# ShardianLabs/EphemeralNet

Measured on AMD Instinct MI355X. Metric: GiB/s ChaCha20-Poly1305 seal+open (device-resident) at 1/2/4/8 MI355X, higher is better.
Workload: dtype u32; 1 GPU; C2: 65536 x 4096 B records, per-record (key, nonce), AEAD seal+open, device-resident; records_per_gpu=65536, record_bytes=4096, lanes_per_record=2, parallelism=records split over 1 GPU(s), no collective

## Files before the change

### ephemeralnet_amd/csrc/enet_device.hpp

```cpp
#pragma once

#include <hip/hip_runtime.h>
#include <stdint.h>

#include "chacha_lockstep_asm.hpp"

namespace enet {

constexpr uint32_t kSigma0 = 0x61707865u, kSigma1 = 0x3320646eu, kSigma2 = 0x79622d32u,
                   kSigma3 = 0x6b206574u;

__device__ __forceinline__ uint32_t rotl(uint32_t v, int s) { return __builtin_rotateleft32(v, s); }

#define ENET_QR(a, b, c, d)                  \
    do {                                     \
        a += b; d ^= a; d = rotl(d, 16);     \
        c += d; b ^= c; b = rotl(b, 12);     \
        a += b; d ^= a; d = rotl(d, 8);      \
        c += d; b ^= c; b = rotl(b, 7);      \
    } while (0)

struct ChachaRecord {
    uint32_t k[8];
    uint32_t n[3];
    uint32_t pre[12];
};

__device__ __forceinline__ void chacha_record_init(ChachaRecord& R, const uint32_t k[8],
                                                   const uint32_t n[3]) {
#pragma unroll
    for (int i = 0; i < 8; ++i) R.k[i] = k[i];
#pragma unroll
    for (int i = 0; i < 3; ++i) R.n[i] = n[i];
    uint32_t a1 = kSigma1, b1 = k[1], c1 = k[5], d1 = n[0];
    uint32_t a2 = kSigma2, b2 = k[2], c2 = k[6], d2 = n[1];
    uint32_t a3 = kSigma3, b3 = k[3], c3 = k[7], d3 = n[2];
    ENET_QR(a1, b1, c1, d1);
    ENET_QR(a2, b2, c2, d2);
    ENET_QR(a3, b3, c3, d3);
    R.pre[0] = a1; R.pre[1] = b1; R.pre[2] = c1; R.pre[3] = d1;
    R.pre[4] = a2; R.pre[5] = b2; R.pre[6] = c2; R.pre[7] = d2;
    R.pre[8] = a3; R.pre[9] = b3; R.pre[10] = c3; R.pre[11] = d3;
}

__device__ __forceinline__ void chacha_block(const ChachaRecord& R, uint32_t counter,
                                             uint32_t x[16]) {
    uint32_t x0 = kSigma0, x4 = R.k[0], x8 = R.k[4], x12 = counter;
    ENET_QR(x0, x4, x8, x12);
    uint32_t x1 = R.pre[0], x5 = R.pre[1], x9 = R.pre[2], x13 = R.pre[3];
    uint32_t x2 = R.pre[4], x6 = R.pre[5], x10 = R.pre[6], x14 = R.pre[7];
    uint32_t x3 = R.pre[8], x7 = R.pre[9], x11 = R.pre[10], x15 = R.pre[11];
    ENET_QR(x0, x5, x10, x15);
    ENET_QR(x1, x6, x11, x12);
    ENET_QR(x2, x7, x8, x13);
    ENET_QR(x3, x4, x9, x14);
#pragma unroll
    for (int i = 1; i < 10; ++i) {
        ENET_QR(x0, x4, x8, x12);
        ENET_QR(x1, x5, x9, x13);
        ENET_QR(x2, x6, x10, x14);
        ENET_QR(x3, x7, x11, x15);
        ENET_QR(x0, x5, x10, x15);
        ENET_QR(x1, x6, x11, x12);
        ENET_QR(x2, x7, x8, x13);
        ENET_QR(x3, x4, x9, x14);
    }
    x[0] = x0 + kSigma0; x[1] = x1 + kSigma1; x[2] = x2 + kSigma2; x[3] = x3 + kSigma3;
    x[4] = x4 + R.k[0]; x[5] = x5 + R.k[1]; x[6] = x6 + R.k[2]; x[7] = x7 + R.k[3];
    x[8] = x8 + R.k[4]; x[9] = x9 + R.k[5]; x[10] = x10 + R.k[6]; x[11] = x11 + R.k[7];
    x[12] = x12 + counter; x[13] = x13 + R.n[0]; x[14] = x14 + R.n[1]; x[15] = x15 + R.n[2];
}

__device__ __forceinline__ void chacha_block2(const ChachaRecord& R, uint32_t ca, uint32_t cb,
                                              uint32_t xa[16], uint32_t xb[16]) {
    uint32_t a0 = kSigma0, a4 = R.k[0], a8 = R.k[4], a12 = ca;
    uint32_t b0 = kSigma0, b4 = R.k[0], b8 = R.k[4], b12 = cb;
    ENET_QR(a0, a4, a8, a12);
    ENET_QR(b0, b4, b8, b12);
    uint32_t a1 = R.pre[0], a5 = R.pre[1], a9 = R.pre[2], a13 = R.pre[3];
    uint32_t a2 = R.pre[4], a6 = R.pre[5], a10 = R.pre[6], a14 = R.pre[7];
    uint32_t a3 = R.pre[8], a7 = R.pre[9], a11 = R.pre[10], a15 = R.pre[11];
    uint32_t b1 = a1, b5 = a5, b9 = a9, b13 = a13;
    uint32_t b2 = a2, b6 = a6, b10 = a10, b14 = a14;
    uint32_t b3 = a3, b7 = a7, b11 = a11, b15 = a15;
    ENET_QR(a0, a5, a10, a15); ENET_QR(b0, b5, b10, b15);
    ENET_QR(a1, a6, a11, a12); ENET_QR(b1, b6, b11, b12);
    ENET_QR(a2, a7, a8, a13);  ENET_QR(b2, b7, b8, b13);
    ENET_QR(a3, a4, a9, a14);  ENET_QR(b3, b4, b9, b14);
#pragma unroll
    for (int i = 1; i < 10; ++i) {
        ENET_QR(a0, a4, a8, a12);  ENET_QR(b0, b4, b8, b12);
        ENET_QR(a1, a5, a9, a13);  ENET_QR(b1, b5, b9, b13);
        ENET_QR(a2, a6, a10, a14); ENET_QR(b2, b6, b10, b14);
        ENET_QR(a3, a7, a11, a15); ENET_QR(b3, b7, b11, b15);
        ENET_QR(a0, a5, a10, a15); ENET_QR(b0, b5, b10, b15);
        ENET_QR(a1, a6, a11, a12); ENET_QR(b1, b6, b11, b12);
        ENET_QR(a2, a7, a8, a13);  ENET_QR(b2, b7, b8, b13);
        ENET_QR(a3, a4, a9, a14);  ENET_QR(b3, b4, b9, b14);
    }
    xa[0] = a0 + kSigma0; xa[1] = a1 + kSigma1; xa[2] = a2 + kSigma2; xa[3] = a3 + kSigma3;
    xa[4] = a4 + R.k[0]; xa[5] = a5 + R.k[1]; xa[6] = a6 + R.k[2]; xa[7] = a7 + R.k[3];
    xa[8] = a8 + R.k[4]; xa[9] = a9 + R.k[5]; xa[10] = a10 + R.k[6]; xa[11] = a11 + R.k[7];
    xa[12] = a12 + ca; xa[13] = a13 + R.n[0]; xa[14] = a14 + R.n[1]; xa[15] = a15 + R.n[2];
    xb[0] = b0 + kSigma0; xb[1] = b1 + kSigma1; xb[2] = b2 + kSigma2; xb[3] = b3 + kSigma3;
    xb[4] = b4 + R.k[0]; xb[5] = b5 + R.k[1]; xb[6] = b6 + R.k[2]; xb[7] = b7 + R.k[3];
    xb[8] = b8 + R.k[4]; xb[9] = b9 + R.k[5]; xb[10] = b10 + R.k[6]; xb[11] = b11 + R.k[7];
    xb[12] = b12 + cb; xb[13] = b13 + R.n[0]; xb[14] = b14 + R.n[1]; xb[15] = b15 + R.n[2];
}

#define ENET_ASM_ADD(x, y) asm volatile("v_add_u32_e32 %0, %0, %1" : "+v"(x) : "v"(y))
#define ENET_ASM_XOR(x, y) asm volatile("v_xor_b32_e32 %0, %0, %1" : "+v"(x) : "v"(y))
#define ENET_ASM_ROT(x, r) asm volatile("v_alignbit_b32 %0, %0, %0, %1" : "+v"(x) : "I"(32 - (r)))

template <bool DIAG>
__device__ __forceinline__ void chacha_half_lockstep(uint32_t x[32]) {
    constexpr int C[4][4] = {{0, 4, 8, 12}, {1, 5, 9, 13}, {2, 6, 10, 14}, {3, 7, 11, 15}};
    constexpr int D[4][4] = {{0, 5, 10, 15}, {1, 6, 11, 12}, {2, 7, 8, 13}, {3, 4, 9, 14}};
    constexpr int R[4] = {16, 12, 8, 7};
#pragma unroll
    for (int k = 0; k < 4; ++k) {
#pragma unroll
        for (int c = 0; c < 8; ++c) {
            const int* q = DIAG ? D[c & 3] : C[c & 3];
            const int o = 16 * (c >> 2);
            if (k % 2 == 0) ENET_ASM_ADD(x[o + q[0]], x[o + q[1]]);
            else ENET_ASM_ADD(x[o + q[2]], x[o + q[3]]);
        }
#pragma unroll
        for (int c = 0; c < 8; ++c) {
            const int* q = DIAG ? D[c & 3] : C[c & 3];
            const int o = 16 * (c >> 2);
            if (k % 2 == 0) ENET_ASM_XOR(x[o + q[3]], x[o + q[0]]);
            else ENET_ASM_XOR(x[o + q[1]], x[o + q[2]]);
        }
#pragma unroll
        for (int c = 0; c < 8; ++c) {
            const int* q = DIAG ? D[c & 3] : C[c & 3];
            const int o = 16 * (c >> 2);
            if (k % 2 == 0) ENET_ASM_ROT(x[o + q[3]], R[k]);
            else ENET_ASM_ROT(x[o + q[1]], R[k]);
        }
#ifndef ENET_LOCK_EVERY
#define ENET_LOCK_EVERY 1
#endif
        if ((k + 1) % ENET_LOCK_EVERY == 0) __builtin_amdgcn_s_barrier();
    }
}

struct NoStepHook {
    __device__ __forceinline__ void operator()(int) const {}
};
template <bool DIAG, class SH = NoStepHook, int BAR = 1>
__device__ __forceinline__ void chacha_half_lockstep2(uint32_t x[32], SH&& sh = SH{}, int base = 0) {
    auto after = [&](int k) {
        asm volatile("" ::: "memory");
        sh(base + k);
        asm volatile("" ::: "memory");
    };
    constexpr bool b0 = BAR == 1, b1 = BAR == 1 || BAR == 2, b2 = BAR == 1, b3 = BAR != 0;
#define ENET_LS_STEP(NAME, B)                               \
    do {                                                    \
        if constexpr (B) asm volatile(NAME ENET_LS_X32(x)); \
        else asm volatile(NAME##_NB ENET_LS_X32(x));        \
    } while (0)
    if constexpr (DIAG) {
        ENET_LS_STEP(ENET_LS_D0, b0);
        after(0);
        ENET_LS_STEP(ENET_LS_D1, b1);
        after(1);
        ENET_LS_STEP(ENET_LS_D2, b2);
        after(2);
        ENET_LS_STEP(ENET_LS_D3, b3);
        after(3);
    } else {
        ENET_LS_STEP(ENET_LS_C0, b0);
        after(0);
        ENET_LS_STEP(ENET_LS_C1, b1);
        after(1);
        ENET_LS_STEP(ENET_LS_C2, b2);
        after(2);
        ENET_LS_STEP(ENET_LS_C3, b3);
        after(3);
    }
#undef ENET_LS_STEP
}

__device__ __forceinline__ void chacha_block2_lockstep(const ChachaRecord& R, uint32_t ca, uint32_t cb,
                                                       uint32_t xa[16], uint32_t xb[16]) {
    uint32_t a0 = kSigma0, a4 = R.k[0], a8 = R.k[4], a12 = ca;
    uint32_t b0 = kSigma0, b4 = R.k[0], b8 = R.k[4], b12 = cb;
    ENET_QR(a0, a4, a8, a12);
    ENET_QR(b0, b4, b8, b12);
    uint32_t x[32];
    x[0] = a0; x[4] = a4; x[8] = a8; x[12] = a12;
    x[16] = b0; x[20] = b4; x[24] = b8; x[28] = b12;
#pragma unroll
    for (int c = 1; c < 4; ++c) {
#pragma unroll
        for (int r = 0; r < 4; ++r) {
            x[c + 4 * r] = R.pre[4 * (c - 1) + r];
            x[16 + c + 4 * r] = R.pre[4 * (c - 1) + r];
        }
    }
    chacha_half_lockstep2<true>(x);
#pragma unroll
    for (int i = 1; i < 10; ++i) {
        chacha_half_lockstep2<false>(x);
        chacha_half_lockstep2<true>(x);
    }
    const uint32_t ff[16] = {kSigma0, kSigma1, kSigma2, kSigma3, R.k[0], R.k[1], R.k[2], R.k[3],
                             R.k[4], R.k[5], R.k[6], R.k[7], 0u, R.n[0], R.n[1], R.n[2]};
#pragma unroll
    for (int i = 0; i < 16; ++i) {
        xa[i] = x[i] + (i == 12 ? ca : ff[i]);
        xb[i] = x[16 + i] + (i == 12 ? cb : ff[i]);
    }
}

constexpr uint32_t M26 = 0x3ffffffu;

struct Pmul {
    uint32_t r[5];
    uint32_t s[5];
};

__device__ __forceinline__ Pmul pmul_make(const uint32_t r[5]) {
    Pmul m;
#pragma unroll
    for (int i = 0; i < 5; ++i) { m.r[i] = r[i]; m.s[i] = r[i] * 5u; }
    return m;
}

__device__ __forceinline__ void pmul(uint32_t h[5], const Pmul& m) {
    const uint64_t h0 = h[0], h1 = h[1], h2 = h[2], h3 = h[3], h4 = h[4];
    uint64_t d0 = h0 * m.r[0] + h1 * m.s[4] + h2 * m.s[3] + h3 * m.s[2] + h4 * m.s[1];
    uint64_t d1 = h0 * m.r[1] + h1 * m.r[0] + h2 * m.s[4] + h3 * m.s[3] + h4 * m.s[2];
    uint64_t d2 = h0 * m.r[2] + h1 * m.r[1] + h2 * m.r[0] + h3 * m.s[4] + h4 * m.s[3];
    uint64_t d3 = h0 * m.r[3] + h1 * m.r[2] + h2 * m.r[1] + h3 * m.r[0] + h4 * m.s[4];
    uint64_t d4 = h0 * m.r[4] + h1 * m.r[3] + h2 * m.r[2] + h3 * m.r[1] + h4 * m.r[0];
    uint32_t c;
    c = (uint32_t)(d0 >> 26); h[0] = (uint32_t)d0 & M26; d1 += c;
    c = (uint32_t)(d1 >> 26); h[1] = (uint32_t)d1 & M26; d2 += c;
    c = (uint32_t)(d2 >> 26); h[2] = (uint32_t)d2 & M26; d3 += c;
    c = (uint32_t)(d3 >> 26); h[3] = (uint32_t)d3 & M26; d4 += c;
    c = (uint32_t)(d4 >> 26); h[4] = (uint32_t)d4 & M26;
    h[0] += c * 5u;
    c = h[0] >> 26; h[0] &= M26; h[1] += c;
}

__device__ __forceinline__ void padd_block(uint32_t h[5], uint32_t w0, uint32_t w1, uint32_t w2,
                                           uint32_t w3, uint32_t hibit) {
    h[0] += w0 & M26;
    h[1] += __builtin_amdgcn_alignbit(w1, w0, 26) & M26;
    h[2] += __builtin_amdgcn_alignbit(w2, w1, 20) & M26;
    h[3] += __builtin_amdgcn_alignbit(w3, w2, 14) & M26;
    h[4] += (w3 >> 8) | (hibit << 24);
}

__device__ __forceinline__ void plimbs(uint32_t out[5], uint32_t w0, uint32_t w1, uint32_t w2,
                                       uint32_t w3) {
    out[0] = w0 & M26;
    out[1] = __builtin_amdgcn_alignbit(w1, w0, 26) & M26;
    out[2] = __builtin_amdgcn_alignbit(w2, w1, 20) & M26;
    out[3] = __builtin_amdgcn_alignbit(w3, w2, 14) & M26;
    out[4] = w3 >> 8;
}

__device__ __forceinline__ void pfinish(const uint32_t hin[5], const uint32_t s[4],
                                        uint32_t tag[4]) {
    uint32_t h0 = hin[0], h1 = hin[1], h2 = hin[2], h3 = hin[3], h4 = hin[4], c;
#pragma unroll
    for (int pass = 0; pass < 2; ++pass) {
        c = h0 >> 26; h0 &= M26; h1 += c;
        c = h1 >> 26; h1 &= M26; h2 += c;
        c = h2 >> 26; h2 &= M26; h3 += c;
        c = h3 >> 26; h3 &= M26; h4 += c;
        c = h4 >> 26; h4 &= M26; h0 += c * 5u;
    }
    c = h0 >> 26; h0 &= M26; h1 += c;
    uint32_t g0 = h0 + 5u; c = g0 >> 26; g0 &= M26;
    uint32_t g1 = h1 + c; c = g1 >> 26; g1 &= M26;
    uint32_t g2 = h2 + c; c = g2 >> 26; g2 &= M26;
    uint32_t g3 = h3 + c; c = g3 >> 26; g3 &= M26;
    uint32_t g4 = h4 + c - (1u << 26);
    const uint32_t use_g = (g4 >> 31) - 1u;
    h0 = (h0 & ~use_g) | (g0 & use_g);
    h1 = (h1 & ~use_g) | (g1 & use_g);
    h2 = (h2 & ~use_g) | (g2 & use_g);
    h3 = (h3 & ~use_g) | (g3 & use_g);
    h4 = (h4 & ~use_g) | (g4 & use_g);
    uint64_t f;
    f = (uint64_t)(h0 | (h1 << 26)) + s[0]; tag[0] = (uint32_t)f;
    f = (uint64_t)((h1 >> 6) | (h2 << 20)) + s[1] + (f >> 32); tag[1] = (uint32_t)f;
    f = (uint64_t)((h2 >> 12) | (h3 << 14)) + s[2] + (f >> 32); tag[2] = (uint32_t)f;
    f = (uint64_t)((h3 >> 18) | (h4 << 8)) + s[3] + (f >> 32); tag[3] = (uint32_t)f;
}

__device__ __forceinline__ void pclamp(uint32_t r[5], uint32_t w0, uint32_t w1, uint32_t w2,
                                       uint32_t w3) {
    plimbs(r, w0 & 0x0fffffffu, w1 & 0x0ffffffcu, w2 & 0x0ffffffcu, w3 & 0x0ffffffcu);
}

struct PolyR32 {
    uint32_t r0, r1, r2, r3, s1, s2, s3;
};

__device__ __forceinline__ PolyR32 polyr32_make(uint32_t w0, uint32_t w1, uint32_t w2, uint32_t w3) {
    PolyR32 R;
    R.r0 = w0 & 0x0fffffffu;
    R.r1 = w1 & 0x0ffffffcu;
    R.r2 = w2 & 0x0ffffffcu;
    R.r3 = w3 & 0x0ffffffcu;
    R.s1 = R.r1 + (R.r1 >> 2);
    R.s2 = R.r2 + (R.r2 >> 2);
    R.s3 = R.r3 + (R.r3 >> 2);
    return R;
}

__device__ __forceinline__ void poly32_block(uint32_t h[5], const PolyR32& R, uint32_t m0,
                                             uint32_t m1, uint32_t m2, uint32_t m3,
                                             uint32_t hibit) {
    unsigned cy;
    const uint32_t a0 = __builtin_addc(h[0], m0, 0u, &cy);
    const uint32_t a1 = __builtin_addc(h[1], m1, cy, &cy);
    const uint32_t a2 = __builtin_addc(h[2], m2, cy, &cy);
    const uint32_t a3 = __builtin_addc(h[3], m3, cy, &cy);
    const uint32_t a4 = h[4] + hibit + cy;
    const uint64_t d0 = (uint64_t)a0 * R.r0 + (uint64_t)a1 * R.s3 + (uint64_t)a2 * R.s2 +
                        (uint64_t)a3 * R.s1;
    const uint64_t e1 = (uint64_t)a0 * R.r1 + (uint64_t)a1 * R.r0 + (uint64_t)a2 * R.s3 +
                        (uint64_t)a3 * R.s2 + (uint64_t)a4 * R.s1;
    const uint64_t e2 = (uint64_t)a0 * R.r2 + (uint64_t)a1 * R.r1 + (uint64_t)a2 * R.r0 +
                        (uint64_t)a3 * R.s3 + (uint64_t)a4 * R.s2;
    const uint64_t e3 = (uint64_t)a0 * R.r3 + (uint64_t)a1 * R.r2 + (uint64_t)a2 * R.r1 +
                        (uint64_t)a3 * R.r0 + (uint64_t)a4 * R.s3;
    const uint32_t x0 = (uint32_t)d0;
    const uint32_t x1 = __builtin_addc((uint32_t)e1, (uint32_t)(d0 >> 32), 0u, &cy);
    const uint32_t c1 = (uint32_t)(e1 >> 32) + cy;
    const uint32_t x2 = __builtin_addc((uint32_t)e2, c1, 0u, &cy);
    const uint32_t c2 = (uint32_t)(e2 >> 32) + cy;
    const uint32_t x3 = __builtin_addc((uint32_t)e3, c2, 0u, &cy);
    const uint32_t c3 = (uint32_t)(e3 >> 32) + cy;
    const uint32_t t4 = a4 * R.r0 + c3;
    const uint32_t f = (t4 >> 2) * 5u;
    h[0] = __builtin_addc(x0, f, 0u, &cy);
    h[1] = __builtin_addc(x1, 0u, cy, &cy);
    h[2] = __builtin_addc(x2, 0u, cy, &cy);
    h[3] = __builtin_addc(x3, 0u, cy, &cy);
    h[4] = (t4 & 3u) + cy;
}

__device__ __forceinline__ void h32_to_limbs(const uint32_t h[5], uint32_t l[5]) {
    l[0] = h[0] & M26;
    l[1] = __builtin_amdgcn_alignbit(h[1], h[0], 26) & M26;
    l[2] = __builtin_amdgcn_alignbit(h[2], h[1], 20) & M26;
    l[3] = __builtin_amdgcn_alignbit(h[3], h[2], 14) & M26;
    l[4] = (h[3] >> 8) | (h[4] << 24);
}

__device__ __forceinline__ void ppow(const uint32_t r[5], uint32_t e, uint32_t x[5]) {
#pragma unroll
    for (int i = 0; i < 5; ++i) x[i] = r[i];
    const Pmul mr = pmul_make(r);
    const int top = 31 - __builtin_clz(e);
    for (int b = top - 1; b >= 0; --b) {
        pmul(x, pmul_make(x));
        if ((e >> b) & 1u) pmul(x, mr);
    }
}

__device__ __forceinline__ uint32_t bswap32(uint32_t v) { return __builtin_bswap32(v); }
__device__ __forceinline__ uint32_t rotr(uint32_t v, int s) { return __builtin_rotateright32(v, s); }

__constant__ static const uint32_t kSha256K[64] = {
    0x428a2f98u, 0x71374491u, 0xb5c0fbcfu, 0xe9b5dba5u, 0x3956c25bu, 0x59f111f1u, 0x923f82a4u,
    0xab1c5ed5u, 0xd807aa98u, 0x12835b01u, 0x243185beu, 0x550c7dc3u, 0x72be5d74u, 0x80deb1feu,
    0x9bdc06a7u, 0xc19bf174u, 0xe49b69c1u, 0xefbe4786u, 0x0fc19dc6u, 0x240ca1ccu, 0x2de92c6fu,
    0x4a7484aau, 0x5cb0a9dcu, 0x76f988dau, 0x983e5152u, 0xa831c66du, 0xb00327c8u, 0xbf597fc7u,
    0xc6e00bf3u, 0xd5a79147u, 0x06ca6351u, 0x14292967u, 0x27b70a85u, 0x2e1b2138u, 0x4d2c6dfcu,
    0x53380d13u, 0x650a7354u, 0x766a0abbu, 0x81c2c92eu, 0x92722c85u, 0xa2bfe8a1u, 0xa81a664bu,
    0xc24b8b70u, 0xc76c51a3u, 0xd192e819u, 0xd6990624u, 0xf40e3585u, 0x106aa070u, 0x19a4c116u,
    0x1e376c08u, 0x2748774cu, 0x34b0bcb5u, 0x391c0cb3u, 0x4ed8aa4au, 0x5b9cca4fu, 0x682e6ff3u,
    0x748f82eeu, 0x78a5636fu, 0x84c87814u, 0x8cc70208u, 0x90befffau, 0xa4506cebu, 0xbef9a3f7u,
    0xc67178f2u};

constexpr uint32_t kShaIV[8] = {0x6a09e667u, 0xbb67ae85u, 0x3c6ef372u, 0xa54ff53au,
                                0x510e527fu, 0x9b05688cu, 0x1f83d9abu, 0x5be0cd19u};

__device__ __forceinline__ uint32_t xor3(uint32_t a, uint32_t b, uint32_t c) {
    return __builtin_amdgcn_bitop3_b32(a, b, c, 0x96);
}

__device__ __forceinline__ void sha256_compress(uint32_t st[8], uint32_t w[16]) {
    uint32_t a = st[0], b = st[1], c = st[2], d = st[3], e = st[4], f = st[5], g = st[6],
             h = st[7];
#pragma unroll
    for (int i = 0; i < 64; ++i) {
        uint32_t wi;
        if (i < 16) {
            wi = w[i];
        } else {
            const uint32_t w15 = w[(i - 15) & 15], w2 = w[(i - 2) & 15];
            const uint32_t s0 = xor3(rotr(w15, 7), rotr(w15, 18), w15 >> 3);
            const uint32_t s1 = xor3(rotr(w2, 17), rotr(w2, 19), w2 >> 10);
            wi = w[i & 15] + s0 + w[(i - 7) & 15] + s1;
            w[i & 15] = wi;
        }
        const uint32_t S1 = xor3(rotr(e, 6), rotr(e, 11), rotr(e, 25));
        const uint32_t ch = __builtin_amdgcn_bitop3_b32(e, f, g, 0xCA);
        const uint32_t t1 = h + S1 + ch + kSha256K[i] + wi;
        const uint32_t S0 = xor3(rotr(a, 2), rotr(a, 13), rotr(a, 22));
        const uint32_t mj = __builtin_amdgcn_bitop3_b32(a, b, c, 0xE8);
        h = g; g = f; f = e; e = d + t1; d = c; c = b; b = a; a = t1 + S0 + mj;
    }
    st[0] += a; st[1] += b; st[2] += c; st[3] += d;
    st[4] += e; st[5] += f; st[6] += g; st[7] += h;
}

template <int N, int M>
__device__ __forceinline__ void extract_bytes(const uint32_t* in, uint32_t off, uint32_t* out) {
    constexpr int W = N + 1;
    uint32_t a[W];
#pragma unroll
    for (int i = 0; i < N; ++i) a[i] = in[i];
    a[N] = 0u;
    const uint32_t k = off >> 2;
#pragma unroll
    for (int b = 32; b >= 1; b >>= 1) {
        if (b > N) continue;
        const bool t = (k & (uint32_t)b) != 0u;
#pragma unroll
        for (int i = 0; i < W; ++i) a[i] = t ? (i + b < W ? a[i + b] : 0u) : a[i];
    }
    const uint32_t sh = off & 3u;
#pragma unroll
    for (int j = 0; j < M; ++j)
        out[j] = __builtin_amdgcn_alignbyte(j + 1 < W ? a[j + 1] : 0u, a[j], sh);
}

__device__ __forceinline__ void load_block(const uint8_t* __restrict__ p, uint32_t n,
                                           uint32_t w[16], bool window_ok = false) {
    if (n >= 64) {
        const uint4* q = reinterpret_cast<const uint4*>(p);
#pragma unroll
        for (int i = 0; i < 4; ++i) {
            const uint4 v = q[i];
            w[4 * i] = v.x; w[4 * i + 1] = v.y; w[4 * i + 2] = v.z; w[4 * i + 3] = v.w;
        }
    } else if (window_ok) {
        const uint32_t nq = n >> 4;
#pragma unroll
        for (int i = 0; i < 16; ++i) w[i] = 0u;
#pragma unroll
        for (int c = 0; c < 3; ++c) {
            if ((uint32_t)c < nq) {
                const uint4 v = reinterpret_cast<const uint4*>(p)[c];
                w[4 * c] = v.x; w[4 * c + 1] = v.y; w[4 * c + 2] = v.z; w[4 * c + 3] = v.w;
            }
        }
        const uint4 v = *reinterpret_cast<const uint4*>(p + n - 16);
        const uint32_t win[4] = {v.x, v.y, v.z, v.w};
        uint32_t ch[4];
        extract_bytes<4, 4>(win, 16u - (n & 15u), ch);
#pragma unroll
        for (int c = 0; c < 4; ++c) {
#pragma unroll
            for (int i = 0; i < 4; ++i) w[4 * c + i] = ((uint32_t)c == nq) ? ch[i] : w[4 * c + i];
        }
    } else {
#pragma unroll
        for (int i = 0; i < 16; ++i) {
            uint32_t v = 0;
#pragma unroll
            for (int b = 0; b < 4; ++b)
                if ((uint32_t)(4 * i + b) < n) v |= (uint32_t)p[4 * i + b] << (8 * b);
            w[i] = v;
        }
    }
}

__device__ __forceinline__ void store_block(uint8_t* __restrict__ p, uint32_t n,
                                            const uint32_t w[16]) {
    if (n >= 64) {
        uint4* q = reinterpret_cast<uint4*>(p);
#pragma unroll
        for (int i = 0; i < 4; ++i)
            q[i] = make_uint4(w[4 * i], w[4 * i + 1], w[4 * i + 2], w[4 * i + 3]);
    } else if (n >= 16) {
        const uint32_t nq = n >> 4;
#pragma unroll
        for (int c = 0; c < 3; ++c)
            if ((uint32_t)c < nq)
                reinterpret_cast<uint4*>(p)[c] =
                    make_uint4(w[4 * c], w[4 * c + 1], w[4 * c + 2], w[4 * c + 3]);
        uint32_t win[4];
        extract_bytes<16, 4>(w, n - 16u, win);
        *reinterpret_cast<uint4*>(p + n - 16) = make_uint4(win[0], win[1], win[2], win[3]);
    } else {
        const uint32_t nw = n >> 2;
#pragma unroll
        for (int i = 0; i < 3; ++i)
            if ((uint32_t)i < nw) *reinterpret_cast<uint32_t*>(p + 4 * i) = w[i];
        const uint32_t lw = nw == 0 ? w[0] : nw == 1 ? w[1] : nw == 2 ? w[2] : w[3];
#pragma unroll
        for (int b = 0; b < 3; ++b)
            if ((uint32_t)b < (n & 3u)) p[4 * nw + b] = (uint8_t)(lw >> (8 * b));
    }
}

__device__ __forceinline__ uint64_t uniform_u64(uint64_t v) {
    return (uint64_t)(uint32_t)__builtin_amdgcn_readfirstlane((uint32_t)v) |
           ((uint64_t)(uint32_t)__builtin_amdgcn_readfirstlane((uint32_t)(v >> 32)) << 32);
}

__device__ __forceinline__ uint32_t ld32(const uint8_t* p) {
    return (uint32_t)p[0] | ((uint32_t)p[1] << 8) | ((uint32_t)p[2] << 16) | ((uint32_t)p[3] << 24);
}

}
```

### ephemeralnet_amd/csrc/stream.hip

```cpp
#include "record_route.hpp"
#include "stream_common.hpp"

namespace enet {

struct StreamSched {
    int dA, dE, sA, sE;
};
__device__ constexpr StreamSched stream_sched(int v) {
    return v == 1 ? StreamSched{1, 2, 2, 2} : v == 2 ? StreamSched{1, 4, 3, 4}
         : v == 3 ? StreamSched{1, 1, 18, 3} : v == 4 ? StreamSched{1, 2, 2, 2}
         : v == 5 ? StreamSched{1, 1, 1, 1} : StreamSched{1, 3, 2, 3};
}
__device__ constexpr int stream_barf(int v) { return v == 4 ? 2 : v == 5 ? 4 : 1; }
__device__ constexpr int stream_stores_after(StreamSched sc) {
    int n = 0;
    for (int s = 0; s < 16; ++s) n += (sc.sA + sc.sE * s >= sc.dA + 15 * sc.dE) ? 1 : 0;
    return n;
}

template <int LOGP, int MODE, int SCHED = 0>
__global__ __launch_bounds__(kStreamWG) void stream_kernel(RecParams p) {
    constexpr StreamSched SC = stream_sched(SCHED);
    constexpr int BARF = stream_barf(SCHED);
    constexpr int kPos = kStreamSteps / BARF;
    constexpr uint32_t P = 1u << LOGP;
    constexpr bool kPoly = (MODE != MODE_XOR);
    __shared__ __attribute__((aligned(16))) uint8_t s_in[kStreamLanes * kRun];
    __shared__ __attribute__((aligned(16))) uint8_t s_out[kStreamLanes * kRun];

    const uint32_t L = (uint32_t)p.uniform_len;
    const bool compute = threadIdx.x < kStreamLanes;
    const uint32_t gid = blockIdx.x * kStreamLanes + (compute ? threadIdx.x : 0u);
    const uint32_t rec = gid >> LOGP;
    const uint32_t j = gid & (P - 1);
#ifdef ENET_TOOLS_BUILD
    const int dbg = p.dbg;
#else
    constexpr int dbg = 0;
#endif
    const bool stamp = (dbg & 16384) && threadIdx.x == 0 && p.tag_out;
    uint64_t* stamps = reinterpret_cast<uint64_t*>(p.tag_out + 16ull * rec);
    if (__builtin_expect(stamp, 0)) {
        stamps[0] = __builtin_amdgcn_s_memrealtime();
        stamps[1] = __builtin_amdgcn_s_memtime();
    }
    const uint64_t i0 = p.in_off[0], o0 = p.out_off[0];
    {
        const bool mine = !compute || (p.in_off[rec] == i0 + (uint64_t)rec * L &&
                                       p.in_off[rec + 1] == i0 + (uint64_t)(rec + 1) * L &&
                                       p.out_off[rec] == o0 + (uint64_t)rec * L &&
                                       p.out_off[rec + 1] == o0 + (uint64_t)(rec + 1) * L);
        if (!__syncthreads_and(mine ? 1 : 0)) {
            if (compute) records_body<LOGP, MODE, FR_NONE, 7>(p);
            return;
        }
    }

    const uint32_t lane = threadIdx.x & 63u;
    const uint32_t wave = __builtin_amdgcn_readfirstlane(threadIdx.x >> 6);
    const uint32_t B = L >> (6 + LOGP);
    const uint32_t S = B >> 1;
    const bool mem = !(dbg & 1);

    if (!compute) {
        const uint32_t m = wave - 8u;
        const uint32_t kk = lane & 7u;
        if (!(dbg & 4096)) __builtin_amdgcn_s_setprio(3);
        uint32_t offA[2], offAB[2];
#pragma unroll
        for (int c = 0; c < 2; ++c) {
            const uint32_t wg0 = blockIdx.x * kStreamLanes + (2u * m + c) * 64u;
            uint32_t o2[2];
#pragma unroll
            for (int i = 0; i < 2; ++i) {
                const uint32_t o = 8u * i + (lane >> 3);
                const uint32_t go = wg0 + o;
                o2[i] = (go >> LOGP) * L + (((go & (P - 1)) * B) << 6) + 16u * (kk ^ slab_sw(o));
            }
            offA[c] = o2[0];
            offAB[c] = o2[1] - o2[0];
        }
        const uint32_t offD = (16u >> LOGP) * L;
        uint32_t offs[16];
#pragma unroll
        for (int s = 0; s < 16; ++s)
            offs[s] = offA[s >> 3] + (uint32_t)(s & 1) * offAB[s >> 3] + (uint32_t)((s & 7) >> 1) * offD;
        auto uni = [](const void* q) {
            const uint64_t v = reinterpret_cast<uintptr_t>(q);
            return (uint64_t)(uint32_t)__builtin_amdgcn_readfirstlane((uint32_t)v) |
                   ((uint64_t)(uint32_t)__builtin_amdgcn_readfirstlane((uint32_t)(v >> 32)) << 32);
        };
        const uint8_t* ibase = reinterpret_cast<const uint8_t*>(uni(p.in + i0));
        uint8_t* obase = reinterpret_cast<uint8_t*>(uni(p.out + o0));
        const uint32_t in_part = (uint32_t)reinterpret_cast<uintptr_t>(s_in) + 2u * m * (64u * kRun);
        const uint8_t* out_part = s_out + 2u * m * (64u * kRun) + 16u * lane;
        auto dma = [&](const uint8_t* base, int s) {
            const uint32_t m0 = in_part + 1024u * (uint32_t)s;
            uint32_t keep;
            if constexpr (SCHED == 14)
                asm volatile("s_mov_b32 %0, m0\n s_mov_b32 m0, %2\n s_nop 0\n global_load_lds_dwordx4 %1, %3\n s_mov_b32 m0, %0"
                             : "=&s"(keep) : "v"(offs[s]), "s"(m0), "s"(base) : "memory");
            else
                asm volatile("s_mov_b32 %0, m0\n s_mov_b32 m0, %2\n s_nop 0\n global_load_lds_dwordx4 %1, %3 nt\n s_mov_b32 m0, %0"
                             : "=&s"(keep) : "v"(offs[s]), "s"(m0), "s"(base) : "memory");
        };
        auto ldsread = [&](int s) {
            return *reinterpret_cast<const uint4*>(out_part + 1024u * (uint32_t)s);
        };
        auto store = [&](uint8_t* base, int s, uint4 v) {
            enet_u32x4 d = {v.x, v.y, v.z, v.w};
            asm volatile("global_store_dwordx4 %0, %1, %2 nt\n s_nop 1"
                         :: "v"(offs[s]), "v"(d), "s"(base) : "memory");
        };
        uint64_t wait_cyc = 0;
        if (mem) {
#pragma unroll
            for (int s = 0; s < 16; ++s) dma(ibase, s);
            asm volatile("s_waitcnt vmcnt(0)" ::: "memory");
        }
        for (uint32_t st = 0; st < S; ++st) {
            stream_barrier();
            const bool more = mem && st + 1 < S && !(dbg & 128), prev = mem && st > 0 && !(dbg & 64);
            const uint8_t* inext = ibase + (size_t)kRun * (st + 1);
            uint8_t* oprev = obase + (size_t)kRun * (st - 1);
            uint4 v = make_uint4(0, 0, 0, 0);
            if (__builtin_expect(prev, 1)) v = ldsread(0);
#pragma unroll
            for (int k = 0; k < kPos; ++k) {
                if (k >= SC.dA && (k - SC.dA) % SC.dE == 0 && (k - SC.dA) / SC.dE < 16) {
                    if (__builtin_expect(more, 1)) dma(inext, (k - SC.dA) / SC.dE);
                }
                if (k >= SC.sA && (k - SC.sA) % SC.sE == 0 && (k - SC.sA) / SC.sE < 16) {
                    const int sl = (k - SC.sA) / SC.sE;
                    if (__builtin_expect(prev, 1)) {
                        store(oprev, sl, v);
                        if (sl < 15) v = ldsread(sl + 1);
                    }
                }
                stream_barrier();
            }
            constexpr int kStoresAfter = stream_stores_after(SC);
            uint64_t tw0 = 0;
            if (__builtin_expect(dbg & 2048, 0)) tw0 = __builtin_amdgcn_s_memtime();
            if (__builtin_expect(prev, 1)) asm volatile("s_waitcnt vmcnt(%0)" :: "n"(kStoresAfter) : "memory");
            else asm volatile("s_waitcnt vmcnt(0)" ::: "memory");
            if (__builtin_expect(dbg & 2048, 0)) wait_cyc += __builtin_amdgcn_s_memtime() - tw0;
        }
        if (__builtin_expect(dbg & 2048, 0) && lane == 0 && p.tag_out)
            reinterpret_cast<uint64_t*>(p.tag_out)[blockIdx.x * 4u + m] = wait_cyc;
        stream_barrier();
        if (S > 0 && mem) {
            uint8_t* olast = obase + (size_t)kRun * (S - 1);
#pragma unroll
            for (int s = 0; s < 16; ++s) store(olast, s, ldsread(s));
        }
        asm volatile("s_waitcnt vmcnt(0)" ::: "memory");
        stream_barrier();
        return;
    }

    const uint32_t msw = slab_sw(lane);
    if (__builtin_expect(stamp, 0)) stamps[2] = __builtin_amdgcn_s_memtime();

    uint32_t kw[8], nw[3];
    {
        const uint32_t* kp = reinterpret_cast<const uint32_t*>(p.keys + (size_t)p.key_stride * rec);
#pragma unroll
        for (int i = 0; i < 8; ++i) kw[i] = kp[i];
        const uint32_t* np = reinterpret_cast<const uint32_t*>(p.nonces + 12ull * rec);
#pragma unroll
        for (int i = 0; i < 3; ++i) nw[i] = np[i];
    }
    ChachaRecord R;
    chacha_record_init(R, kw, nw);
    uint32_t ctr = 1u;
    if (MODE == MODE_XOR)
        ctr = p.counters ? p.counters[(size_t)rec * (p.counter_stride ? p.counter_stride : 1u)] : 0u;
    ctr += j * B;

    uint64_t clk0 = 0, rt0 = 0;
    if (dbg & 256) {
        clk0 = __builtin_amdgcn_s_memtime();
        rt0 = __builtin_amdgcn_s_memrealtime();
    }

    uint32_t h[5] = {0, 0, 0, 0, 0};
    PolyR32 PR{};
    uint32_t pad[4] = {0, 0, 0, 0};
    uint32_t na = 0, aad_len = 0;
    if (kPoly) {
        uint32_t otk[16];
        chacha_block(R, 0u, otk);
        PR = polyr32_make(otk[0], otk[1], otk[2], otk[3]);
        pad[0] = otk[4]; pad[1] = otk[5]; pad[2] = otk[6]; pad[3] = otk[7];
        uint64_t aoff = 0;
        if (p.aad) {
            aoff = p.aad_off[rec];
            aad_len = (uint32_t)(p.aad_off[rec + 1] - aoff);
        }
        na = (aad_len + 15) >> 4;
        if (j == 0) {
            for (uint32_t s = 0; s < na; ++s) {
                const uint8_t* ap = p.aad + aoff + 16ull * s;
                const uint32_t cnt = min(16u, aad_len - 16u * s);
                uint32_t w[4];
#pragma unroll
                for (int i = 0; i < 4; ++i) {
                    uint32_t v = 0;
#pragma unroll
                    for (int b = 0; b < 4; ++b)
                        if ((uint32_t)(4 * i + b) < cnt) v |= (uint32_t)ap[4 * i + b] << (8 * b);
                    w[i] = v;
                }
                poly32_block(h, PR, w[0], w[1], w[2], w[3], 1u);
            }
        }
    }

    const uint32_t ff[16] = {kSigma0, kSigma1, kSigma2, kSigma3, R.k[0], R.k[1], R.k[2], R.k[3],
                             R.k[4], R.k[5], R.k[6], R.k[7], 0u, R.n[0], R.n[1], R.n[2]};
    for (uint32_t st = 0; st < S; ++st) {
        asm volatile("s_waitcnt lgkmcnt(0)" ::: "memory");
        stream_barrier();
        if (__builtin_expect(stamp, 0)) stamps[3 + st] = __builtin_amdgcn_s_memtime();
        uint8_t* myrun = s_in + threadIdx.x * kRun;
        uint32_t w[32];
        if (__builtin_expect(dbg & 32, 0)) {
#pragma unroll
            for (int k = 0; k < 32; ++k) w[k] = k * lane + st;
        } else {
#pragma unroll
            for (int k = 0; k < 8; ++k) {
                const uint4 v = *reinterpret_cast<const uint4*>(myrun + 16u * (k ^ msw));
                w[4 * k] = v.x; w[4 * k + 1] = v.y; w[4 * k + 2] = v.z; w[4 * k + 3] = v.w;
            }
        }
        const uint32_t c0 = ctr + 2u * st;
        uint32_t x[32];
        {
            uint32_t a0 = kSigma0, a4 = R.k[0], a8 = R.k[4], a12 = c0;
            uint32_t b0 = kSigma0, b4 = R.k[0], b8 = R.k[4], b12 = c0 + 1u;
            ENET_QR(a0, a4, a8, a12);
            ENET_QR(b0, b4, b8, b12);
            x[0] = a0; x[4] = a4; x[8] = a8; x[12] = a12;
            x[16] = b0; x[20] = b4; x[24] = b8; x[28] = b12;
#pragma unroll
            for (int c = 1; c < 4; ++c) {
#pragma unroll
                for (int r = 0; r < 4; ++r) {
                    x[c + 4 * r] = R.pre[4 * (c - 1) + r];
                    x[16 + c + 4 * r] = R.pre[4 * (c - 1) + r];
                }
            }
        }
        asm volatile("s_waitcnt lgkmcnt(0)" ::: "memory");
        if (__builtin_expect(dbg & 2, 0)) {
#pragma unroll
            for (int k = 0; k < kPos; ++k) stream_barrier();
        } else {
            chacha_half_lockstep2<true, NoStepHook, BARF>(x);
#pragma unroll
            for (int dr = 1; dr < 10; ++dr) {
                chacha_half_lockstep2<false, NoStepHook, BARF>(x);
                chacha_half_lockstep2<true, NoStepHook, BARF>(x);
            }
        }
        if (MODE == MODE_OPEN && !(dbg & 4)) {
            poly_block64(h, PR, w);
            poly_block64(h, PR, w + 16);
        }
#pragma unroll
        for (int i = 0; i < 16; ++i) {
            w[i] ^= x[i] + (i == 12 ? c0 : ff[i]);
            w[16 + i] ^= x[16 + i] + (i == 12 ? c0 + 1u : ff[i]);
        }
        if (MODE == MODE_SEAL && !(dbg & 4)) {
            poly_block64(h, PR, w);
            poly_block64(h, PR, w + 16);
        }
        uint8_t* myout = s_out + threadIdx.x * kRun;
        if (__builtin_expect(dbg & 32, 0)) {
            uint32_t acc = 0;
#pragma unroll
            for (int k = 0; k < 32; ++k) acc ^= w[k];
            if (acc == 0x9e3779b9u) myout[0] = 1;
        } else {
#pragma unroll
            for (int k = 0; k < 8; ++k)
                *reinterpret_cast<uint4*>(myout + 16u * (k ^ msw)) =
                    make_uint4(w[4 * k], w[4 * k + 1], w[4 * k + 2], w[4 * k + 3]);
        }
    }
    asm volatile("s_waitcnt lgkmcnt(0)" ::: "memory");
    stream_barrier();
    if (__builtin_expect(stamp, 0)) stamps[3 + S] = __builtin_amdgcn_s_memtime();

    if (dbg & (256 | 2048 | 16384)) {
        const uint64_t clk1 = __builtin_amdgcn_s_memtime(), rt1 = __builtin_amdgcn_s_memrealtime();
        if (threadIdx.x == 0 && p.tag_out && !(dbg & (2048 | 16384))) {
            uint64_t* d = reinterpret_cast<uint64_t*>(p.tag_out + 16ull * rec);
            d[0] = clk0; d[1] = rt0; d[2] = clk1; d[3] = rt1;
        }
        stream_barrier();
        if (__builtin_expect(stamp, 0)) {
            stamps[4 + S] = __builtin_amdgcn_s_memtime();
            stamps[5 + S] = __builtin_amdgcn_s_memrealtime();
        }
        return;
    }
    uint32_t diff = 0;
    if (kPoly) {
        const uint32_t nct = L >> 4;
        const uint32_t N = na + nct + 1;
        uint32_t e = 0;
        if (j == P - 1) poly32_block(h, PR, aad_len, 0u, L, 0u, 1u);
        else e = N - 1 - (na + 4 * (j + 1) * B - 1);
        uint32_t l[5];
        h32_to_limbs(h, l);
        if (P > 1) {
            if (e > 0) {
                uint32_t r26[5], xx[5];
                plimbs(r26, PR.r0, PR.r1, PR.r2, PR.r3);
                ppow(r26, e, xx);
                pmul(l, pmul_make(xx));
            }
#pragma unroll
            for (uint32_t o = P >> 1; o >= 1; o >>= 1) {
#pragma unroll
                for (int i = 0; i < 5; ++i) l[i] += __shfl_xor(l[i], (int)o);
            }
        }
        uint32_t tag[4];
        pfinish(l, pad, tag);
        if (MODE == MODE_SEAL) {
            if (j == 0) {
                uint32_t* tp = reinterpret_cast<uint32_t*>(p.tag_out + 16ull * rec);
                tp[0] = tag[0]; tp[1] = tag[1]; tp[2] = tag[2]; tp[3] = tag[3];
            }
        } else {
            const uint32_t* tp = reinterpret_cast<const uint32_t*>(p.tag_in + 16ull * rec);
            diff = (tag[0] ^ tp[0]) | (tag[1] ^ tp[1]) | (tag[2] ^ tp[2]) | (tag[3] ^ tp[3]);
            if (j == 0) p.ok[rec] = diff == 0 ? 1 : 0;
        }
    }
    stream_barrier();
    if (MODE == MODE_OPEN && diff != 0) {
        uint8_t* seg = p.out + o0 + (uint64_t)rec * L + ((uint64_t)j * B << 6);
        for (uint32_t c = 0; c < 4 * B; ++c)
            *reinterpret_cast<uint4*>(seg + 16ull * c) = make_uint4(0, 0, 0, 0);
    }
}

template <int MODE>
static hipError_t launch_stream_mode(const RecParams& p, uint32_t lanes, uint32_t blocks, hipStream_t s) {
    switch (lanes) {
        case 1: hipLaunchKernelGGL((stream_kernel<0, MODE>), dim3(blocks), dim3(kStreamWG), 0, s, p); break;
        case 2:
#ifdef ENET_TOOLS_BUILD
            switch (p.var) {
                case 1: hipLaunchKernelGGL((stream_kernel<1, MODE, 1>), dim3(blocks), dim3(kStreamWG), 0, s, p); break;
                case 2: hipLaunchKernelGGL((stream_kernel<1, MODE, 2>), dim3(blocks), dim3(kStreamWG), 0, s, p); break;
                case 3: hipLaunchKernelGGL((stream_kernel<1, MODE, 3>), dim3(blocks), dim3(kStreamWG), 0, s, p); break;
                case 4: hipLaunchKernelGGL((stream_kernel<1, MODE, 4>), dim3(blocks), dim3(kStreamWG), 0, s, p); break;
                case 5: hipLaunchKernelGGL((stream_kernel<1, MODE, 5>), dim3(blocks), dim3(kStreamWG), 0, s, p); break;
                case 14: hipLaunchKernelGGL((stream_kernel<1, MODE, 14>), dim3(blocks), dim3(kStreamWG), 0, s, p); break;
                default: hipLaunchKernelGGL((stream_kernel<1, MODE>), dim3(blocks), dim3(kStreamWG), 0, s, p); break;
            }
#else
            hipLaunchKernelGGL((stream_kernel<1, MODE>), dim3(blocks), dim3(kStreamWG), 0, s, p);
#endif
            break;
        case 4: hipLaunchKernelGGL((stream_kernel<2, MODE>), dim3(blocks), dim3(kStreamWG), 0, s, p); break;
        case 8: hipLaunchKernelGGL((stream_kernel<3, MODE>), dim3(blocks), dim3(kStreamWG), 0, s, p); break;
        case 16: hipLaunchKernelGGL((stream_kernel<4, MODE>), dim3(blocks), dim3(kStreamWG), 0, s, p); break;
        default: return hipErrorInvalidValue;
    }
    return hipGetLastError();
}

static_assert(kRouteWideWG == kStreamLanes, "record_route.hpp and the streaming kernel disagree on the workgroup");

hipError_t launch_stream(int mode, const RecParams& p, uint32_t lanes, uint32_t blocks, hipStream_t s) {
    switch (mode) {
        case MODE_XOR: return launch_stream_mode<MODE_XOR>(p, lanes, blocks, s);
        case MODE_SEAL: return launch_stream_mode<MODE_SEAL>(p, lanes, blocks, s);
        case MODE_OPEN: return launch_stream_mode<MODE_OPEN>(p, lanes, blocks, s);
        default: return hipErrorInvalidValue;
    }
}

}
```

### ephemeralnet_amd/csrc/stream_common.hpp

```cpp
#pragma once
#include "records_body.hpp"

namespace enet {

constexpr uint32_t kStreamLanes = 512;
constexpr uint32_t kStreamWG = 768;
constexpr int kStreamSteps = 76;

__device__ __forceinline__ void stream_barrier() { asm volatile("s_barrier" ::: "memory"); }

}
```

Before: 912.7 GiB/s.

## Interleave Poly1305 pieces into ChaCha lockstep steps and add wave-priority variants

Adds a PolySpreadHook that breaks each Poly1305 block update into nine pieces and runs them between the ChaCha lockstep quarter-round steps in open mode. The aim is to hide the MAC arithmetic inside the ChaCha schedule instead of running poly_block64 afterwards. It also adds configurable s_setprio variants for the compute and memory waves, plus a debug timing probe. The default build (issue variant 30) keeps the sequential poly path but pins the w registers first; the spread and priority variants are selectable only in tools builds. The cost is extra register pressure and compiler barriers from the pinning.

```diff
diff --git a/ephemeralnet_amd/csrc/enet_device.hpp b/ephemeralnet_amd/csrc/enet_device.hpp
--- a/ephemeralnet_amd/csrc/enet_device.hpp
+++ b/ephemeralnet_amd/csrc/enet_device.hpp
@@ -2,6 +2,9 @@
 
 #include <hip/hip_runtime.h>
 #include <stdint.h>
+
+#include <type_traits>
+#include <utility>
 
 #include "chacha_lockstep_asm.hpp"
 
@@ -150,11 +153,11 @@
 struct NoStepHook {
     __device__ __forceinline__ void operator()(int) const {}
 };
-template <bool DIAG, class SH = NoStepHook, int BAR = 1>
-__device__ __forceinline__ void chacha_half_lockstep2(uint32_t x[32], SH&& sh = SH{}, int base = 0) {
-    auto after = [&](int k) {
+template <bool DIAG, class SH = NoStepHook, int BAR = 1, int BASE = 0>
+__device__ __forceinline__ void chacha_half_lockstep2(uint32_t x[32], SH&& sh = SH{}) {
+    auto after = [&](auto k) {
         asm volatile("" ::: "memory");
-        sh(base + k);
+        sh(std::integral_constant<int, BASE + decltype(k)::value>{});
         asm volatile("" ::: "memory");
     };
     constexpr bool b0 = BAR == 1, b1 = BAR == 1 || BAR == 2, b2 = BAR == 1, b3 = BAR != 0;
@@ -165,22 +168,22 @@
     } while (0)
     if constexpr (DIAG) {
         ENET_LS_STEP(ENET_LS_D0, b0);
-        after(0);
+        after(std::integral_constant<int, 0>{});
         ENET_LS_STEP(ENET_LS_D1, b1);
-        after(1);
+        after(std::integral_constant<int, 1>{});
         ENET_LS_STEP(ENET_LS_D2, b2);
-        after(2);
+        after(std::integral_constant<int, 2>{});
         ENET_LS_STEP(ENET_LS_D3, b3);
-        after(3);
+        after(std::integral_constant<int, 3>{});
     } else {
         ENET_LS_STEP(ENET_LS_C0, b0);
-        after(0);
+        after(std::integral_constant<int, 0>{});
         ENET_LS_STEP(ENET_LS_C1, b1);
-        after(1);
+        after(std::integral_constant<int, 1>{});
         ENET_LS_STEP(ENET_LS_C2, b2);
-        after(2);
+        after(std::integral_constant<int, 2>{});
         ENET_LS_STEP(ENET_LS_C3, b3);
-        after(3);
+        after(std::integral_constant<int, 3>{});
     }
 #undef ENET_LS_STEP
 }
diff --git a/ephemeralnet_amd/csrc/stream.hip b/ephemeralnet_amd/csrc/stream.hip
--- a/ephemeralnet_amd/csrc/stream.hip
+++ b/ephemeralnet_amd/csrc/stream.hip
@@ -12,10 +12,32 @@
          : v == 5 ? StreamSched{1, 1, 1, 1} : StreamSched{1, 3, 2, 3};
 }
 __device__ constexpr int stream_barf(int v) { return v == 4 ? 2 : v == 5 ? 4 : 1; }
+#ifndef ENET_STREAM_ISSUE
+#define ENET_STREAM_ISSUE 30
+#endif
+struct StreamIssue {
+    int prio_old, prio_young, prio_mem, poly;
+};
+__device__ constexpr StreamIssue stream_issue(int v) {
+    int k = -1, poly = 0;
+    if (v >= 20 && v < 28) k = v - 20;
+    else if (v >= 30 && v <= 32) poly = v - 29;
+    if (k < 0) return StreamIssue{0, 0, 3, poly};
+    const int c = k & 3;
+    return StreamIssue{c == 0 ? 0 : c == 3 ? 2 : 1, c == 1 ? 0 : c == 3 ? 2 : 1, (k & 4) ? 2 : 3, poly};
+}
 __device__ constexpr int stream_stores_after(StreamSched sc) {
     int n = 0;
     for (int s = 0; s < 16; ++s) n += (sc.sA + sc.sE * s >= sc.dA + 15 * sc.dE) ? 1 : 0;
     return n;
+}
+
+__device__ __forceinline__ void stream_where(const RecParams& p, int logp, uint32_t wave, uint32_t lane,
+                                             uint64_t t_entry) {
+    if (lane != 0 || !p.tag_out) return;
+    const uint32_t hw = __builtin_amdgcn_s_getreg(4 | (31 << 11));
+    uint32_t* d = reinterpret_cast<uint32_t*>(p.tag_out + 16ull * ((blockIdx.x * kStreamLanes) >> logp) + 16u * wave);
+    d[0] = (uint32_t)t_entry; d[1] = (uint32_t)(t_entry >> 32); d[2] = hw; d[3] = wave;
 }
 
 template <int LOGP, int MODE, int SCHED = 0>
@@ -25,6 +47,7 @@
     constexpr int kPos = kStreamSteps / BARF;
     constexpr uint32_t P = 1u << LOGP;
     constexpr bool kPoly = (MODE != MODE_XOR);
+    constexpr StreamIssue ISS = stream_issue(SCHED < 20 ? ENET_STREAM_ISSUE : SCHED);
     __shared__ __attribute__((aligned(16))) uint8_t s_in[kStreamLanes * kRun];
     __shared__ __attribute__((aligned(16))) uint8_t s_out[kStreamLanes * kRun];
 
@@ -39,6 +62,8 @@
     constexpr int dbg = 0;
 #endif
     const bool stamp = (dbg & 16384) && threadIdx.x == 0 && p.tag_out;
+    uint64_t t_entry = 0;
+    if (__builtin_expect(dbg & 32768, 0)) t_entry = __builtin_amdgcn_s_memtime();
     uint64_t* stamps = reinterpret_cast<uint64_t*>(p.tag_out + 16ull * rec);
     if (__builtin_expect(stamp, 0)) {
         stamps[0] = __builtin_amdgcn_s_memrealtime();
@@ -65,7 +90,7 @@
     if (!compute) {
         const uint32_t m = wave - 8u;
         const uint32_t kk = lane & 7u;
-        if (!(dbg & 4096)) __builtin_amdgcn_s_setprio(3);
+        if (!(dbg & 4096)) __builtin_amdgcn_s_setprio(ISS.prio_mem);
         uint32_t offA[2], offAB[2];
 #pragma unroll
         for (int c = 0; c < 2; ++c) {
@@ -156,6 +181,7 @@
         }
         asm volatile("s_waitcnt vmcnt(0)" ::: "memory");
         stream_barrier();
+        if (__builtin_expect(dbg & 32768, 0)) stream_where(p, LOGP, wave, lane, t_entry);
         return;
     }
 
@@ -219,6 +245,13 @@
 
     const uint32_t ff[16] = {kSigma0, kSigma1, kSigma2, kSigma3, R.k[0], R.k[1], R.k[2], R.k[3],
                              R.k[4], R.k[5], R.k[6], R.k[7], 0u, R.n[0], R.n[1], R.n[2]};
+    if constexpr (ISS.prio_old == ISS.prio_young) {
+        if constexpr (ISS.prio_old != 0) __builtin_amdgcn_s_setprio(ISS.prio_old);
+    } else if (wave >= 4u) {
+        if constexpr (ISS.prio_young != 0) __builtin_amdgcn_s_setprio(ISS.prio_young);
+    } else {
+        if constexpr (ISS.prio_old != 0) __builtin_amdgcn_s_setprio(ISS.prio_old);
+    }
     for (uint32_t st = 0; st < S; ++st) {
         asm volatile("s_waitcnt lgkmcnt(0)" ::: "memory");
         stream_barrier();
@@ -257,6 +290,15 @@
         if (__builtin_expect(dbg & 2, 0)) {
 #pragma unroll
             for (int k = 0; k < kPos; ++k) stream_barrier();
+        } else if constexpr (MODE == MODE_OPEN && ISS.poly >= 2) {
+            using Hook = PolySpreadHook<ISS.poly == 2>;
+            constexpr int HB = ISS.poly == 2 ? 0 : 1;
+            Hook hook(h, PR, w);
+            chacha_half_lockstep2<true, Hook&, HB, 0>(x, hook);
+            [&]<int... DR>(std::integer_sequence<int, DR...>) {
+                ((chacha_half_lockstep2<false, Hook&, HB, 8 * DR + 4>(x, hook),
+                  chacha_half_lockstep2<true, Hook&, HB, 8 * DR + 8>(x, hook)), ...);
+            }(std::make_integer_sequence<int, 9>{});
         } else {
             chacha_half_lockstep2<true, NoStepHook, BARF>(x);
 #pragma unroll
@@ -265,7 +307,11 @@
                 chacha_half_lockstep2<true, NoStepHook, BARF>(x);
             }
         }
-        if (MODE == MODE_OPEN && !(dbg & 4)) {
+        if constexpr (MODE == MODE_OPEN && ISS.poly == 1) {
+#pragma unroll
+            for (int i = 0; i < 32; ++i) ENET_PIN(w[i]);
+        }
+        if (MODE == MODE_OPEN && ISS.poly < 2 && !(dbg & 4)) {
             poly_block64(h, PR, w);
             poly_block64(h, PR, w + 16);
         }
@@ -295,9 +341,9 @@
     stream_barrier();
     if (__builtin_expect(stamp, 0)) stamps[3 + S] = __builtin_amdgcn_s_memtime();
 
-    if (dbg & (256 | 2048 | 16384)) {
+    if (dbg & (256 | 2048 | 16384 | 32768)) {
         const uint64_t clk1 = __builtin_amdgcn_s_memtime(), rt1 = __builtin_amdgcn_s_memrealtime();
-        if (threadIdx.x == 0 && p.tag_out && !(dbg & (2048 | 16384))) {
+        if (threadIdx.x == 0 && p.tag_out && !(dbg & (2048 | 16384 | 32768))) {
             uint64_t* d = reinterpret_cast<uint64_t*>(p.tag_out + 16ull * rec);
             d[0] = clk0; d[1] = rt0; d[2] = clk1; d[3] = rt1;
         }
@@ -306,6 +352,7 @@
             stamps[4 + S] = __builtin_amdgcn_s_memtime();
             stamps[5 + S] = __builtin_amdgcn_s_memrealtime();
         }
+        if (dbg & 32768) stream_where(p, LOGP, wave, lane, t_entry);
         return;
     }
     uint32_t diff = 0;
@@ -352,6 +399,11 @@
 }
 
 template <int MODE>
+constexpr int stream_issue_var(int v) {
+    return (MODE == MODE_OPEN || v < 30) ? v : 0;
+}
+
+template <int MODE>
 static hipError_t launch_stream_mode(const RecParams& p, uint32_t lanes, uint32_t blocks, hipStream_t s) {
     switch (lanes) {
         case 1: hipLaunchKernelGGL((stream_kernel<0, MODE>), dim3(blocks), dim3(kStreamWG), 0, s, p); break;
@@ -364,6 +416,10 @@
                 case 4: hipLaunchKernelGGL((stream_kernel<1, MODE, 4>), dim3(blocks), dim3(kStreamWG), 0, s, p); break;
                 case 5: hipLaunchKernelGGL((stream_kernel<1, MODE, 5>), dim3(blocks), dim3(kStreamWG), 0, s, p); break;
                 case 14: hipLaunchKernelGGL((stream_kernel<1, MODE, 14>), dim3(blocks), dim3(kStreamWG), 0, s, p); break;
+#define ENET_VAR(V) case V: hipLaunchKernelGGL((stream_kernel<1, MODE, stream_issue_var<MODE>(V)>), dim3(blocks), dim3(kStreamWG), 0, s, p); break;
+                ENET_VAR(20) ENET_VAR(21) ENET_VAR(22) ENET_VAR(23) ENET_VAR(24) ENET_VAR(25) ENET_VAR(26) ENET_VAR(27)
+                ENET_VAR(30) ENET_VAR(31) ENET_VAR(32)
+#undef ENET_VAR
                 default: hipLaunchKernelGGL((stream_kernel<1, MODE>), dim3(blocks), dim3(kStreamWG), 0, s, p); break;
             }
 #else
diff --git a/ephemeralnet_amd/csrc/stream_common.hpp b/ephemeralnet_amd/csrc/stream_common.hpp
--- a/ephemeralnet_amd/csrc/stream_common.hpp
+++ b/ephemeralnet_amd/csrc/stream_common.hpp
@@ -1,4 +1,6 @@
 #pragma once
+#include <type_traits>
+
 #include "records_body.hpp"
 
 namespace enet {
@@ -9,4 +11,87 @@
 
 __device__ __forceinline__ void stream_barrier() { asm volatile("s_barrier" ::: "memory"); }
 
+#define ENET_PIN(v) asm volatile("" : "+v"(v))
+
+template <bool BAR_AFTER>
+struct PolySpreadHook {
+    uint32_t (&h)[5];
+    const PolyR32& R;
+    const uint32_t (&w)[32];
+    uint32_t a0 = 0, a1 = 0, a2 = 0, a3 = 0, a4 = 0, x0 = 0, x1 = 0, x2 = 0, x3 = 0, c = 0, t4 = 0, f = 0;
+    uint64_t d0 = 0, e1 = 0, e2 = 0, e3 = 0;
+
+    __device__ __forceinline__ PolySpreadHook(uint32_t (&h_)[5], const PolyR32& R_, const uint32_t (&w_)[32])
+        : h(h_), R(R_), w(w_) {}
+
+    __device__ __forceinline__ void pin_a() {
+        ENET_PIN(a0); ENET_PIN(a1); ENET_PIN(a2); ENET_PIN(a3); ENET_PIN(a4);
+    }
+    template <int S>
+    __device__ __forceinline__ void piece() {
+        constexpr int b = 4 * ((S % 72) / 9), q = S < 72 ? S % 9 : -1;
+        unsigned cy;
+        if constexpr (q == 0) {
+            ENET_PIN(h[0]); ENET_PIN(h[1]); ENET_PIN(h[2]); ENET_PIN(h[3]); ENET_PIN(h[4]);
+            a0 = __builtin_addc(h[0], w[b], 0u, &cy);
+            a1 = __builtin_addc(h[1], w[b + 1], cy, &cy);
+            a2 = __builtin_addc(h[2], w[b + 2], cy, &cy);
+            a3 = __builtin_addc(h[3], w[b + 3], cy, &cy);
+            a4 = h[4] + 1u + cy;
+            ENET_PIN(a0); ENET_PIN(a1); ENET_PIN(a2); ENET_PIN(a3); ENET_PIN(a4);
+        } else if constexpr (q == 1) {
+            pin_a();
+            d0 = (uint64_t)a0 * R.r0 + (uint64_t)a1 * R.s3 + (uint64_t)a2 * R.s2 + (uint64_t)a3 * R.s1;
+            ENET_PIN(d0);
+        } else if constexpr (q == 2) {
+            pin_a();
+            e1 = (uint64_t)a0 * R.r1 + (uint64_t)a1 * R.r0 + (uint64_t)a2 * R.s3 + (uint64_t)a3 * R.s2 +
+                 (uint64_t)a4 * R.s1;
+            ENET_PIN(e1);
+        } else if constexpr (q == 3) {
+            pin_a();
+            e2 = (uint64_t)a0 * R.r2 + (uint64_t)a1 * R.r1 + (uint64_t)a2 * R.r0 + (uint64_t)a3 * R.s3 +
+                 (uint64_t)a4 * R.s2;
+            ENET_PIN(e2);
+        } else if constexpr (q == 4) {
+            pin_a();
+            e3 = (uint64_t)a0 * R.r3 + (uint64_t)a1 * R.r2 + (uint64_t)a2 * R.r1 + (uint64_t)a3 * R.r0 +
+                 (uint64_t)a4 * R.s3;
+            ENET_PIN(e3);
+        } else if constexpr (q == 5) {
+            ENET_PIN(d0); ENET_PIN(e1); ENET_PIN(e2);
+            x0 = (uint32_t)d0;
+            x1 = __builtin_addc((uint32_t)e1, (uint32_t)(d0 >> 32), 0u, &cy);
+            c = (uint32_t)(e1 >> 32) + cy;
+            x2 = __builtin_addc((uint32_t)e2, c, 0u, &cy);
+            c = (uint32_t)(e2 >> 32) + cy;
+            ENET_PIN(x1); ENET_PIN(x2); ENET_PIN(c);
+        } else if constexpr (q == 6) {
+            ENET_PIN(e3); ENET_PIN(c); ENET_PIN(a4);
+            x3 = __builtin_addc((uint32_t)e3, c, 0u, &cy);
+            c = (uint32_t)(e3 >> 32) + cy;
+            t4 = a4 * R.r0 + c;
+            ENET_PIN(x3); ENET_PIN(t4);
+        } else if constexpr (q == 7) {
+            ENET_PIN(t4);
+            f = (t4 >> 2) * 5u;
+            t4 &= 3u;
+            ENET_PIN(f); ENET_PIN(t4);
+        } else if constexpr (q == 8) {
+            ENET_PIN(x0); ENET_PIN(x1); ENET_PIN(x2); ENET_PIN(x3); ENET_PIN(f); ENET_PIN(t4);
+            h[0] = __builtin_addc(x0, f, 0u, &cy);
+            h[1] = __builtin_addc(x1, 0u, cy, &cy);
+            h[2] = __builtin_addc(x2, 0u, cy, &cy);
+            h[3] = __builtin_addc(x3, 0u, cy, &cy);
+            h[4] = t4 + cy;
+            ENET_PIN(h[0]); ENET_PIN(h[1]); ENET_PIN(h[2]); ENET_PIN(h[3]); ENET_PIN(h[4]);
+        }
+    }
+    template <int S>
+    __device__ __forceinline__ void operator()(std::integral_constant<int, S>) {
+        piece<S>();
+        if (BAR_AFTER) stream_barrier();
+    }
+};
+
 }
```

Result: faster. 929.2 GiB/s, median of 6 (+1.8%).
